# intel/QAT-ZSTD-Plugin

Measured on AMD Instinct MI355X. Metric: input MB/s via ZSTD_compress2 L1 128KiB blocks @1/2/4/8 GPU; ratio vs sw zstd, higher is better.
Workload: dtype u8

## Files before the change

### qat-zstd-plugin_amd/csrc/qzstd_kernels.hip

```cpp
#include <hip/hip_runtime.h>

#include <stdint.h>
#include <stdio.h>
#include <stdlib.h>
#include <string.h>

#include <atomic>
#include <mutex>
#include <sched.h>
#include <time.h>

#include "qzstd_hip.h"
#include "qzstd_hip_internal.h"

#define QZ_PRIO(n) do { if (!CHAIN) __builtin_amdgcn_s_setprio(n); } while (0)

#ifndef QZ_PARSE_SPLIT
#define QZ_PARSE_SPLIT 3
#endif
#ifndef QZ_LINKS_PER_STEP
#define QZ_LINKS_PER_STEP 4
#endif
#ifndef QZ_WAVES_PER_EU
#define QZ_WAVES_PER_EU 5
#endif
#define QZ_OCCUPANCY __attribute__((amdgpu_waves_per_eu(QZ_WAVES_PER_EU)))

#ifdef QZ_DEBUG_DUMP
#define QZ_PLAP(acc) { const u64 tN = __builtin_amdgcn_s_memtime(); acc += tN - tQ; tQ = tN; }
#define QZ_LAP(acc) { const u64 tN = __builtin_amdgcn_s_memtime(); acc += tN - tP; tP = tN; }
#define QZ_CLAP(k) { const u64 tN = __builtin_amdgcn_s_memtime(); dC[k] += tN - tC; tC = tN; }
#else
#define QZ_PLAP(acc)
#define QZ_LAP(acc)
#define QZ_CLAP(k)
#endif

namespace {

constexpr int kMatchWaves = 8;
constexpr int kMatchThreads = kMatchWaves * 64;
constexpr int kThreads = kMatchThreads + 64;
constexpr uint32_t kTileLog = 9;
constexpr uint32_t kTile = 1u << kTileLog;
constexpr uint32_t kWin = kTile >> 6;
constexpr uint32_t kTagBits = 14;
constexpr uint32_t kTagMask = (1u << kTagBits) - 1u;
constexpr uint32_t kPrime1 = 2654435761u;
constexpr uint32_t kPrime2 = 0x85EBCA77u;
constexpr uint32_t kNone = 0xFFFFFFFFu;
constexpr uint32_t kRing = QZ_RING;
constexpr uint32_t kRingMask = kRing - 1u;
constexpr uint32_t kMirror = QZSTD_HIP_RING_MIRROR;
constexpr uint32_t kLook = 4608u;
constexpr uint32_t kNear = kRing - kLook - 3u * kTile - 1024u;
static_assert((kRing & kRingMask) == 0u && kRing >= 16384u, "the ring is a power of two of at least 16 KiB");
constexpr size_t kLdsPerCu = QZSTD_HIP_LDS_MAX;
constexpr uint32_t kEL = QZSTD_HIP_CHAIN_ENTRY_LINKS;
constexpr uint32_t kEQ = QZSTD_HIP_CHAIN_ENTRY_LINKS / 4u;
static_assert(kEL == 4u || kEL == 8u, "chain entries hold four or eight links");
constexpr uint32_t kLdsBase = QZSTD_HIP_LDS_BASE;
constexpr uint32_t kLagT = 2u;

struct LaunchArgs {
    const uint8_t *src;
    const qzstd_hip_block_t *blocks;
    uint4 *seqs;
    uint32_t *nseq;
    qzstd_hip_profile_t prof;
    uint4 *chain;
    uint32_t chainStride;
    uint32_t chainEntries;
    uint32_t pwWords;
    uint32_t orderedLds;
#ifdef QZ_DEBUG_DUMP
    uint32_t dbg;
#endif
};

// ... 613 lines not shown
        stv[k] = (p < nh && p + 4u <= segE) ? (__umulhi(mixH, pf.tableSize) | (((mixH >> 3) & kTagMask) << 16)) : kNone;
    }
    if (ordered) {
#pragma unroll
        for (uint32_t k = 0; k < kWin; k++) {
            const uint32_t mineK = ((t0 + 64u * k + lane + 1u) << kTagBits) | (stv[k] >> 16);
            uint32_t pred = 0u;
            if (stv[k] != kNone) pred = atomicMax(&tbl[stv[k] & 0xFFFFu], mineK);
            P1[64u * k + lane] = pred;
        }
    } else {
#pragma unroll 1
        for (uint32_t k = 0; k < kWin; k++) {
            const uint32_t st = stv[k];
            const bool vk = st != kNone;
            const uint32_t slotK = st & 0xFFFFu;
            const uint32_t mineK = ((t0 + 64u * k + lane + 1u) << kTagBits) | (st >> 16);
            uint32_t prd = 0u, fin = mineK;
            if (vk) {
                uint32_t *e = &tbl[slotK];
                prd = __hip_atomic_load(e, __ATOMIC_RELAXED, __HIP_MEMORY_SCOPE_WORKGROUP);
                atomicMax(e, mineK);
                fin = __hip_atomic_load(e, __ATOMIC_RELAXED, __HIP_MEMORY_SCOPE_WORKGROUP);
            }
            u64 rem = __ballot(fin != mineK);
            uint32_t predLane = lane;
            while (rem) {
                const uint32_t s0 = rdlane(slotK, (uint32_t)__builtin_ctzll(rem));
                const bool in = vk && slotK == s0;
                const u64 grp = __ballot(in);
                const u64 lower = grp & below(lane);
                if (in && lower) predLane = 63u - (uint32_t)__builtin_clzll(lower);
                rem &= ~grp;
            }
            const uint32_t fromLane = (uint32_t)__shfl((int)mineK, (int)predLane);
            P1[64u * k + lane] = vk ? (predLane != lane ? fromLane : prd) : 0u;
        }
    }
}

struct HistShare {
    uint32_t *flags;
    uint32_t item;
    uint32_t epoch;
    uint32_t spinLimit;
    uint32_t nItems;
    uint32_t *tabFlags;
    uint32_t *linkFlags;
    uint32_t *tabs;
};
constexpr uint32_t kSvcTabStride = QZ_CHAIN_TABLE;
static_assert((uint32_t)kMatchWaves * kPvStride <= QZ_CHAIN_TABLE, "the deferred parse's eight windows of parse words must fit in the head table (QZ_CHAIN_TABLE)");

template <bool HAS_LONG, bool REP, bool CHAIN, bool TURNS, bool NEAR, bool DEFER = false>
__device__ __forceinline__ uint32_t qz_item(const LaunchArgs &args, const qzstd_hip_block_t &blk, const uint8_t *gsrc, uint4 *out,
                                            uint4 *chainB, uint32_t *p1B, const HistShare hsh)
{
    extern __shared__ __attribute__((aligned(16))) uint8_t smem[];
    const uint32_t tid = threadIdx.x;
    const uint32_t lane = tid & 63u;
    const uint32_t wave = rdfirst(tid >> 6);
    const bool matcher = wave < (uint32_t)kMatchWaves;
    const uint32_t n = blk.srcLen;
    const qzstd_hip_profile_t pf = args.prof;
    const uint32_t nh = n >= pf.hashBytes ? n - pf.hashBytes + 1u : 0u;
    const uint32_t nTiles = (nh + kTile - 1u) >> kTileLog;
    const uint32_t itEnd = (DEFER && !CHAIN) ? nTiles : nTiles + kLagT;
    static_assert(kNear + kLagT * kTile + 4u <= kRing - kLook, "the ring no longer holds a near source when its tile is parsed / emitted");
    const uint32_t tabShift = (uint32_t)__builtin_clz(pf.tableSize) + 1u, longShift = pf.longSize ? (uint32_t)__builtin_clz(pf.longSize) + 1u : 31u;
    const uint32_t firstTile = blk.parseFrom >> kTileLog;
    if (blk.parseFrom != 0u && (pf.segLog == 0u || (blk.parseFrom & ((1u << pf.segLog) - 1u)) != 0u || blk.parseFrom >= n)) {
        return QZSTD_HIP_NSEQ_ERROR;
    }
    if (NEAR && n > kRing) return QZSTD_HIP_NSEQ_ERROR;
    if (DEFER && args.pwWords != 0u && ((n + kTile - 1u) & ~(kTile - 1u)) > args.pwWords) return QZSTD_HIP_NSEQ_ERROR;
    if (DEFER && CHAIN && args.chainEntries != 0u && ((n + kTile - 1u) & ~(kTile - 1u)) * kEQ > args.chainEntries) return QZSTD_HIP_NSEQ_ERROR;

    uint8_t *smemI = (uint8_t *)(__attribute__((address_space(3))) uint8_t *)kLdsBase;
    if ((uint32_t)(uintptr_t)(__attribute__((address_space(3))) uint8_t *)smem != 0u) {
        return QZSTD_HIP_NSEQ_ERROR;
    }
    uint32_t *ring32 = reinterpret_cast<uint32_t *>(smemI);
    uint4 *ring128 = reinterpret_cast<uint4 *>(smemI);
    uint32_t *tbl = reinterpret_cast<uint32_t *>(smemI + kRing + kMirror);
    uint32_t *tblL = tbl + pf.tableSize;
    uint32_t *nearTab = tblL + pf.longSize;
    uint32_t *srec = nearTab + kTile;
    uint32_t *pv = srec + kLagT * kWin * kSrecWords;
    uint32_t *turnCtr = pv + kLagT * kPvStride;
    uint32_t *P1odd = turnCtr + QZSTD_HIP_LDS_CTRL / 4u;
    const uint4 *g128 = reinterpret_cast<const uint4 *>(gsrc);
    Src src;
    src.ring = (LdsWords)ring32;
    src.g = (HbmWords)reinterpret_cast<const uint32_t *>(gsrc);
    src.nearLimit = NEAR ? 0xFFFFFFFFu : kNear;
    const uint32_t nPad = (n + 15u) & ~15u;

    const uint32_t itBegin = firstTile;
    const uint32_t histEnd = itBegin << kTileLog;
    const uint32_t hi = umin(nPad, histEnd + kLook + (itBegin ? 0u : kTile));
    const uint32_t lo = hi > kRing ? (hi - kRing + 15u) & ~15u : 0u;
    constexpr uint32_t kStep = (uint32_t)kThreads * 16u;
    const uint32_t hashEnd = CHAIN ? 0u : histEnd;
    uint32_t fo = (hashEnd ? 0u : lo) + tid * 16u;
    uint4 fa0 = make_uint4(0u, 0u, 0u, 0u), fb0 = fa0, fa1 = fa0, fb1 = fa0;
    if (fo < hi) { fa0 = g128[fo >> 4]; if (fo < hashEnd) fb0 = g128[(fo >> 4) + 1u]; }
    if (fo + kStep < hi) { fa1 = g128[(fo + kStep) >> 4]; if (fo + kStep < hashEnd) fb1 = g128[((fo + kStep) >> 4) + 1u]; }
    for (uint32_t i = tid; i < pf.tableSize + pf.longSize; i += kThreads) tbl[i] = 0u;
    if (!(CHAIN && itBegin != 0u)) {
        for (uint32_t i = tid; i < kTile; i += kThreads) nearTab[i] = 0xFFFFFFFFu;
// ... 645 lines not shown
                uint32_t P[9], pa[8];
                load_dw_r<9>(src, p + 16u, rp16, false, P);
#pragma unroll
                for (int i = 0; i < 8; i++) pa[i] = __builtin_amdgcn_alignbyte(P[i + 1], P[i], p & 3u);
                if (need1) { const uint32_t l = tail_len(src, pa, q1 + 16u, ring_back(rp16, p - q1), far1); l1 = 16u + l; need1 = l == 32u && 48u < cap; }
                if (HAS_LONG && need3) { const uint32_t l = tail_len(src, pa, q3 + 16u, ring_back(rp16, p - q3), far3); l3 = 16u + l; need3 = l == 32u && 48u < cap; }
                if (need2) { const uint32_t l = tail_len(src, pa, q2 + 16u, ring_back(rp16, p - q2), false); l2 = 16u + l; need2 = l == 32u && 48u < cap; }
            }
            while (need1 || need2 || need3) {
                const int which = need1 ? 1 : (need3 ? 3 : 2);
                const uint32_t q = which == 1 ? q1 : (which == 3 ? q3 : q2);
                const uint32_t L = which == 1 ? l1 : (which == 3 ? l3 : l2);
                const uint32_t l = chunk_len(src, p + L, ring_fwd(rp, L), p - q, which == 1 ? far1 : (which == 3 ? far3 : false));
                const bool more = l == 32u && L + 32u < cap;
                if (which == 1) { l1 = L + l; need1 = more; }
                else if (which == 3) { l3 = L + l; need3 = more; }
                else { l2 = L + l; need2 = more; }
            }
            QZ_PRIO(0);
            l1 = umin(l1, cap); l2 = umin(l2, cap); l3 = umin(l3, cap);
            if (l1 >= 4u) { cl = l1; off = p - q1; }
            if (l3 >= 4u && l3 > cl) { cl = l3; off = p - q3; }
            if (l2 >= 4u && l2 >= cl) { cl = l2; off = p - q2; }
            }
        }
        }
        if (!CHAIN && it < nTiles && !history && !QZ_ABLATED(4u)) write_flags(it, cl, off);
#pragma unroll
        for (uint32_t i = kLagT - 1u; i > 0u; i--) { offH[i] = offH[i - 1u]; lenH[i] = lenH[i - 1u]; }
        offH[0] = off;
        lenH[0] = cl;
        rp = ring_fwd(rp, kTile);
        QZ_LAP(dI2)
        if (DEFER && !CHAIN) QZ_BARRIER_LDS(); else __syncthreads();
        QZ_LAP(dW2)
    }
#ifdef QZ_DEBUG_DUMP
    if (!(blk.mark & QZSTD_HIP_MARK_COMPACT)) {
    if (lane == 0) out[blk.seqCap - 3u - wave] = make_uint4((uint32_t)dI1, (uint32_t)dW1, (uint32_t)dI2, (uint32_t)dW2);
    if (lane == 0) out[blk.seqCap - 24u - 2u * wave] = make_uint4((uint32_t)(dC[0] >> 4), (uint32_t)(dC[1] >> 4), (uint32_t)(dC[2] >> 4), (uint32_t)(dC[3] >> 4));
    if (lane == 0) out[blk.seqCap - 25u - 2u * wave] = make_uint4((uint32_t)(dC[4] >> 4), (uint32_t)dC[5], 0u, 0u);
    if (lane == 0) out[blk.seqCap - 12u - wave] = make_uint4(__builtin_amdgcn_s_getreg((4 << 0) | (0 << 6) | (31 << 11)), 0u, 0u, 0u);
    }
#endif
    if constexpr (!DEFER) return 0u;
    }

    if constexpr (DEFER && !REP) {
        constexpr uint32_t kSegLog = 12u, kSeg = 1u << kSegLog, kMaxSegs = QZSTD_HIP_BLOCK_MAX >> kSegLog;
        static_assert(kMaxSegs <= 64u, "one lane per segment in the prefix step");
        constexpr uint32_t kNoAnchor = 0xFFFFFFFFu;
        uint32_t *segCnt = srec, *segEndA = srec + kMaxSegs;
        const uint32_t firstSeg = blk.parseFrom >> kSegLog, nSegs = (nh + kSeg - 1u) >> kSegLog;
#ifdef QZ_DEBUG_DUMP
        const u64 tD0 = __builtin_amdgcn_s_memtime();
#endif
        if (wave == 0u && lane == 0u) segCnt[2u * kMaxSegs] = firstSeg;
        __syncthreads();
#ifdef QZ_DEBUG_DUMP
        const u64 tD1 = __builtin_amdgcn_s_memtime();
#endif
        {
            const uint32_t S0 = rdfirst(segCnt[2u * kMaxSegs]);
            const uint32_t lastDw = (nPad >> 2) - 1u;
            auto load_tile = [&](uint32_t tb, uint32_t (&dst)[kWin]) {
#pragma unroll
                for (uint32_t j = 0; j < kWin; j++) dst[j] = p1B[tb + 64u * j + lane];
            };
            uint32_t nxt[kWin];
            uint32_t sgN = S0 + wave;
            if (sgN < nSegs) load_tile(sgN << kSegLog, nxt);
            while (sgN < nSegs) {
                const uint32_t sg = sgN;
                sgN = sg + (uint32_t)kMatchWaves;
                const uint32_t segStart = sg << kSegLog;
                u64 *recG = reinterpret_cast<u64 *>(p1B + segStart);
                const uint32_t tEnd = umin(segStart + kSeg, nTiles << kTileLog);
                PlainParse st = { segStart, 0u, kNoAnchor };
                for (uint32_t base = segStart; base < tEnd; base += kTile) {
                    uint32_t wds[kWin];
#pragma unroll
                    for (uint32_t j = 0; j < kWin; j++) wds[j] = nxt[j];
                    const uint32_t nb = base + kTile < tEnd ? base + kTile : sgN << kSegLog;
                    if (base + kTile < tEnd || sgN < nSegs) load_tile(nb, nxt);
                    parse_plain_windows<0, kWin>(pf, src, recG, base, n, lastDw, lane, wds, st);
                }
                if (lane == 0u) { segCnt[sg] = st.cnt; segEndA[sg] = st.endA; }
            }
        }
#ifdef QZ_DEBUG_DUMP
        const u64 tD2 = __builtin_amdgcn_s_memtime();
#endif
        __syncthreads();
#ifdef QZ_DEBUG_DUMP
        const u64 tD3 = __builtin_amdgcn_s_memtime();
#endif
        const bool mine = lane >= firstSeg && lane < nSegs;
        const uint32_t cv = mine ? segCnt[lane] : 0u, ev = mine ? segEndA[lane] : kNoAnchor;
        uint32_t incl = cv, last = ev;
#pragma unroll
        for (uint32_t d = 1; d < kMaxSegs; d <<= 1) {
            const uint32_t ci = (uint32_t)__shfl_up((int)incl, d), li = (uint32_t)__shfl_up((int)last, d);
            if (lane >= d) { incl += ci; if (last == kNoAnchor) last = li; }
        }
        const uint32_t total = rdlane(incl, kMaxSegs - 1u), lastAll = rdlane(last, kMaxSegs - 1u);
        const uint32_t anchorEndAll = lastAll == kNoAnchor ? blk.parseFrom : lastAll;
        {
            for (uint32_t sg = firstSeg + wave; sg < nSegs; sg += (uint32_t)kMatchWaves) {
                const u64 *recG = reinterpret_cast<const u64 *>(p1B + (sg << kSegLog));
                const uint32_t cnt = rdlane(cv, sg), first = rdlane(incl, sg) - cnt;
                uint32_t anchorIn = blk.parseFrom;
                if (sg > 0u) { const uint32_t a = rdlane(last, sg - 1u); if (a != kNoAnchor) anchorIn = a; }
                constexpr uint32_t kU = 4u;
                for (uint32_t k0 = 0; k0 < cnt; k0 += 64u * kU) {
                    u64 r[kU], rp1[kU];
#pragma unroll
                    for (uint32_t u = 0; u < kU; u++) {
                        const uint32_t k = k0 + 64u * u + lane;
                        r[u] = k < cnt ? recG[k] : 0ull;
                        rp1[u] = (k < cnt && k) ? recG[k - 1u] : 0ull;
                    }
                    uint32_t P0[kU], P1[kU], Q0[kU], Q1[kU], lit[kU], maxb[kU];
#pragma unroll
                    for (uint32_t u = 0; u < kU; u++) {
                        const uint32_t k = k0 + 64u * u + lane;
                        const uint32_t pm = (uint32_t)r[u] & 0x1FFFFu, off = (uint32_t)(r[u] >> 17) & 0x1FFFFu;
                        lit[u] = k ? pm - (((uint32_t)rp1[u] & 0x1FFFFu) + ((uint32_t)(rp1[u] >> 34) & 0x1FFFu))
                                   : pm - anchorIn;
                        const uint32_t q = pm - off;
                        maxb[u] = k < cnt ? umin(umin(umin(pf.backExt, lit[u]), q), pm & (kSeg - 1u)) : 0u;
                        P0[u] = P1[u] = Q0[u] = Q1[u] = 0u;
                        if (maxb[u]) {
                            const uint32_t pa = pm >= 4u ? pm - 4u : 0u, qa = q >= 4u ? q - 4u : 0u;
                            P0[u] = src.g[pa >> 2]; P1[u] = src.g[(pa >> 2) + 1u];
                            Q0[u] = src.g[qa >> 2]; Q1[u] = src.g[(qa >> 2) + 1u];
                        }
                    }
#pragma unroll
                    for (uint32_t u = 0; u < kU; u++) {
                        const uint32_t k = k0 + 64u * u + lane;
                        if (k < cnt) {
                            const uint32_t pm = (uint32_t)r[u] & 0x1FFFFu, off = (uint32_t)(r[u] >> 17) & 0x1FFFFu, len = (uint32_t)(r[u] >> 34) & 0x1FFFu;
                            const uint32_t q = pm - off;
                            uint32_t b = 0;
                            if (maxb[u]) {
                                const uint32_t pa = pm >= 4u ? pm - 4u : 0u, qa = q >= 4u ? q - 4u : 0u;
                                uint32_t pb = __builtin_amdgcn_alignbyte(P1[u], P0[u], pa & 3u), qb = __builtin_amdgcn_alignbyte(Q1[u], Q0[u], qa & 3u);
                                if (pm < 4u) pb <<= 8u * (4u - pm);
                                if (q < 4u) qb <<= 8u * (4u - q);
                                const uint32_t x = pb ^ qb;
                                b = umin(x ? (uint32_t)__builtin_clz(x) >> 3 : 4u, maxb[u]);
                            }
                            const uint32_t idx = first + k;
                            if (idx < blk.seqCap) store_entry(out, idx, off, lit[u] - b, len + b, blk.mark);
                        }
                    }
                }
            }
#ifdef QZ_DEBUG_DUMP
            if (lane == 0 && !(blk.mark & QZSTD_HIP_MARK_COMPACT))
                out[blk.seqCap - 44u - wave] = make_uint4((uint32_t)(tD1 - tD0), (uint32_t)(tD2 - tD1), (uint32_t)(tD3 - tD2), (uint32_t)(__builtin_amdgcn_s_memtime() - tD3));
#endif
        }
        if (wave != 0u) return 0u;
        uint32_t count = total + 1u;
        if (lane == 0 && total < blk.seqCap) store_entry(out, total, 0u, n - anchorEndAll, 0u, blk.mark);
        if (count + 1u >= blk.seqCap) count = QZSTD_HIP_NSEQ_ERROR;
        return count;
    }

    if constexpr (DEFER && REP) {
        constexpr uint32_t kSegLog = 12u, kSeg = 1u << kSegLog, kSegsPerQ = kRing >> kSegLog;
        static_assert(kSegsPerQ == (uint32_t)kMatchWaves, "one wave per segment of a quarter");
        constexpr uint32_t kNoAnchor = 0xFFFFFFFFu;
        __syncthreads();
        uint32_t *pvW = tbl + wave * kPvStride;
        uint32_t *ctl = srec;
        const uint32_t firstSeg = blk.parseFrom >> kSegLog, nSegs = (nh + kSeg - 1u) >> kSegLog;
        uint32_t total = 0u, anchorCarry = blk.parseFrom;
        for (uint32_t Q = firstSeg / kSegsPerQ; Q * kSegsPerQ < nSegs; Q++) {
            const uint32_t qs = Q * kRing;
            for (uint32_t o = qs + tid * 16u; o < umin(qs + kRing, nPad); o += (uint32_t)kMatchThreads * 16u) {
                const uint4 v = g128[o >> 4];
                ring128[(o & kRingMask) >> 4] = v;
                if ((o & kRingMask) < kMirror) ring128[(kRing + (o & kRingMask)) >> 4] = v;
            }
            __syncthreads();
            const uint32_t sg = Q * kSegsPerQ + wave;
            const uint32_t segStart = sg << kSegLog;
            u64 *recG = reinterpret_cast<u64 *>(p1B + segStart);
            uint32_t cnt = 0u, endA = kNoAnchor;
            if (sg >= firstSeg && sg < nSegs) {
                const uint32_t tEnd = umin(segStart + kSeg, nTiles << kTileLog);
                uint32_t nxt[kWin];
#pragma unroll
                for (uint32_t j = 0; j < kWin; j++) nxt[j] = p1B[segStart + 64u * j + lane];
                {
                    RepState st = { segStart, segStart, 0u, 0u, 0u, 0u, sg };
                    for (uint32_t base = segStart; base < tEnd; base += kTile) {
#pragma unroll
                        for (uint32_t j = 0; j < kWin; j++) pvW[64u * j + lane] = nxt[j];
                        if (base + kTile < tEnd) {
#pragma unroll
                            for (uint32_t j = 0; j < kWin; j++) nxt[j] = p1B[base + kTile + 64u * j + lane];
                        }
                        parse_rep_span<true>(pf, src, pvW, base, base + kTile, n, nh, lane, st, qs, recG);
                    }
                    cnt = st.nseq;
                    if (cnt) endA = st.anchor;
                }
            }
            if (lane == 0u) { ctl[wave] = cnt; ctl[kSegsPerQ + wave] = endA; }
            __syncthreads();
            {
                const uint32_t cv = lane < 2u * kSegsPerQ ? ctl[lane] : 0u;
                uint32_t before = 0u, all = 0u, anchorIn = anchorCarry, anchorOut = anchorCarry;
#pragma unroll
                for (uint32_t j = 0; j < kSegsPerQ; j++) {
                    const uint32_t c = rdlane(cv, j), a = rdlane(cv, kSegsPerQ + j);
                    if (j < wave) { before += c; if (a != kNoAnchor) anchorIn = a; }
                    all += c;
                    if (a != kNoAnchor) anchorOut = a;
                }
                const uint32_t cnt = rdlane(cv, wave);
                for (uint32_t k0 = 0; k0 < cnt; k0 += 64u) {
                    const uint32_t k = k0 + lane;
                    if (k < cnt) {
                        const u64 r = recG[k];
                        const uint32_t pm = (uint32_t)r & 0x1FFFFu, off = (uint32_t)(r >> 17) & 0x1FFFFu, len = (uint32_t)(r >> 34) & 0x1FFFu;
                        uint32_t lit = pm - anchorIn;
                        if (k) lit = (uint32_t)(r >> 47) & 0x1FFFu;
                        const uint32_t q = pm - off;
                        const uint32_t maxb = umin(umin(umin(pf.backExt, lit), q), pm & (kSeg - 1u));
                        uint32_t b = 0;
                        if (maxb) {
                            const uint32_t pb = rd32u(src, pm - 4u, false);
                            uint32_t qb;
                            if (q < qs + 4u) qb = q >= 4u ? rd32u(src, q - 4u, true) : rd32u(src, 0u, true) << (8u * (4u - q));
                            else qb = rd32u(src, q - 4u, false);
                            const uint32_t x = pb ^ qb;
                            b = umin(x ? (uint32_t)__builtin_clz(x) >> 3 : 4u, maxb);
                        }
                        const uint32_t idx = total + before + k;
                        if (idx < blk.seqCap) store_entry(out, idx, off, lit - b, len + b, blk.mark);
                    }
                }
                total += all;
                anchorCarry = anchorOut;
            }
            __syncthreads();
        }
        if (wave != 0u) return 0u;
        uint32_t count = total + 1u;
        if (lane == 0 && total < blk.seqCap) store_entry(out, total, 0u, n - anchorCarry, 0u, blk.mark);
        if (count + 1u >= blk.seqCap) count = QZSTD_HIP_NSEQ_ERROR;
        return count;
    }
    return 0u;
}

template <bool HAS_LONG, bool REP, bool CHAIN, bool TURNS, bool NEAR>
__global__ __launch_bounds__(kThreads) QZ_OCCUPANCY void qzstd_find_sequences_kernel(LaunchArgs args)
{
    const qzstd_hip_block_t blk = args.blocks[blockIdx.x];
    const uint32_t count = qz_item<HAS_LONG, REP, CHAIN, TURNS, NEAR, true>(args, blk, args.src + blk.srcOff, args.seqs + blk.seqOff,
                                                              CHAIN ? args.chain + (size_t)blockIdx.x * args.chainStride : nullptr,
                                                              reinterpret_cast<uint32_t *>(args.chain + (size_t)blockIdx.x * args.chainStride + args.chainEntries),
                                                              HistShare{ nullptr, 0u, 0u, 0u, 0u, nullptr, nullptr, nullptr });
    asm volatile("s_waitcnt vmcnt(0)" ::: "memory");
    __syncthreads();
    if (threadIdx.x == 0u)
        __hip_atomic_store(args.nseq + blockIdx.x, count, __ATOMIC_RELEASE, __HIP_MEMORY_SCOPE_SYSTEM);
}

constexpr uint32_t kSvcQueue = 4096u;
constexpr uint32_t kSvcRing = 256u;
constexpr uint32_t kSvcMaxItems = 32u;
constexpr uint32_t kSvcSlots = 1024u;
constexpr uint32_t kSvcRejected = 0xFFFFFFFEu;

struct SvcDev {
    u64 items[kSvcQueue][8];
    uint32_t head;
    uint32_t done;
    uint32_t quit;
    uint32_t spinFails;
    uint32_t started;
    uint32_t taken;
    uint32_t pad[2];
    uint32_t sliceFlag[kSvcSlots][kSvcMaxItems];
    uint32_t histFlag[kSvcSlots][kSvcMaxItems];
    uint32_t tabFlag[kSvcSlots][kSvcMaxItems];
    uint32_t linkFlag[kSvcSlots][kSvcMaxItems];
};

struct SvcHost {
    u64 ring[kSvcRing][8];
    uint32_t state;
    uint32_t quitReq;
    u64 consumed;
    u64 itemsDone;
    uint32_t spinFails;
    uint32_t pad;
    u64 dbg[8];
};

typedef __attribute__((address_space(1))) u64 *gu64p;
typedef __attribute__((address_space(1))) uint32_t *gu32p;

__device__ __forceinline__ u64 svc_tag(u64 n, uint32_t entries) { return (n / entries) % 255ull + 1ull; }
__device__ __forceinline__ u64 svc_payload(u64 g) { return g & 0x00FFFFFFFFFFFFFFull; }


constexpr uint32_t kSvcProfiles = 24u;
__device__ __forceinline__ uint32_t svc_profile_index(uint32_t levelByte) { return ((levelByte & 0x7Fu) - 1u) + ((levelByte & 0x80u) ? 12u : 0u); }

template <bool HAS_LONG, bool REP, bool CHAIN, bool TURNS, bool MULTI>
__global__ __launch_bounds__(kThreads) void qzstd_service_worker(LaunchArgs args, SvcDev *sv, uint32_t ctlOff, uint32_t spinLimit, const qzstd_hip_profile_t *profs)
{
    const uint32_t tid = threadIdx.x, lane = tid & 63u;
    const uint32_t wave = rdfirst(tid >> 6);
    uint32_t *ctl = (uint32_t *)(__attribute__((address_space(3))) uint32_t *)(size_t)(kLdsBase + ctlOff);
    if (tid == 0u) (void)__hip_atomic_fetch_add(&sv->started, 1u, QZ_RLX_AGENT);
    for (;;) {
        if (wave == 0u) {
// ... 244 lines not shown
    hipEvent_t bigEv[kBig] = {};
    bool bigUsed[kBig] = {};
    size_t bigLds[kBig] = {};
    int bigNext = 0;
    size_t lds = 0;
    long long launchNs = 0;
    bool sawWorkers = false;
    bool wide = false;
};
Service g_svc[64];
std::atomic<int> g_svcFreeze{0};

struct SvcConfig { int enabled, workers, idleUs, spinLimit; };
const SvcConfig &svc_config()
{
    static const SvcConfig c = [] {
        SvcConfig k;
        const char *e = getenv("QZSTD_HIP_SERVICE"), *w = getenv("QZSTD_HIP_SERVICE_WORKERS"), *i = getenv("QZSTD_HIP_SERVICE_IDLE_US");
        k.enabled = e ? atoi(e) : 1;
        k.workers = w ? atoi(w) : 0;
        k.idleUs = i ? atoi(i) : 20000;
        if (k.idleUs < 100) k.idleUs = 100;
        k.spinLimit = 1 << 20;
        return k;
    }();
    return c;
}

int svc_stop_locked(Service &s, unsigned waitMs)
{
    if (!s.hs) return 0;
    if (__atomic_load_n(&s.hs->state, __ATOMIC_ACQUIRE) != 0u) {
        __atomic_store_n(&s.hs->quitReq, 1u, __ATOMIC_RELEASE);
        struct timespec t0, t;
        clock_gettime(CLOCK_MONOTONIC, &t0);
        while (__atomic_load_n(&s.hs->state, __ATOMIC_ACQUIRE) != 0u) {
            clock_gettime(CLOCK_MONOTONIC, &t);
            if ((t.tv_sec - t0.tv_sec) * 1000ll + (t.tv_nsec - t0.tv_nsec) / 1000000ll > (long long)waitMs) { s.broken = 1; return 1; }
            sched_yield();
        }
    }
    return 0;
}

#define QZ_SEARCHES(X, last)                                                                                    \
    X(false, false, false, false, last), X(false, true, false, false, last),        \
    X(false, false, false, true, last), X(false, true, false, true, last),                \
    X(false, false, true, true, last), X(false, true, true, true, last),      \
    X(true, false, false, false, last), X(true, true, false, false, last)
#define QZ_K(L, R, C, T, N) reinterpret_cast<const void *>(qzstd_find_sequences_kernel<L, R, C, T, N>)
#define QZ_W(L, R, C, T, M) reinterpret_cast<const void *>(qzstd_service_worker<L, R, C, T, M>)
const void *const kLaunchKernels[16] = { QZ_SEARCHES(QZ_K, false), QZ_SEARCHES(QZ_K, true) };
const void *const kWorkers[8] = { QZ_SEARCHES(QZ_W, false) };
#undef QZ_K
#undef QZ_W
#undef QZ_SEARCHES

int variant_index(const qzstd_hip_profile_t &p, bool nearK)
{
    const int search = p.chainDepth ? 2 : (p.longSize ? 3 : (p.subTileLog ? 1 : 0));
    return (nearK ? 8 : 0) + 2 * search + (p.repWin ? 1 : 0);
}

}

SvcFreeze::SvcFreeze()
{
    g_svcFreeze.fetch_add(1);
    for (int d = 0; d < 64; d++) {
        Service &s = g_svc[d];
        if (!s.hs) continue;
        std::lock_guard<std::mutex> g(s.mu);
        (void)svc_stop_locked(s, 2000);
    }
}
SvcFreeze::~SvcFreeze() { g_svcFreeze.fetch_sub(1); }

static int g_ldsOrdered[64];
static std::mutex g_probeMu;

int probe_lds_order(int device, int physDev)
{
    {
        const int known = __atomic_load_n(&g_ldsOrdered[device], __ATOMIC_ACQUIRE);
        if (known > 0) return known - 1;
    }
    std::lock_guard<std::mutex> g(g_probeMu);
    if (g_ldsOrdered[device] > 0) return g_ldsOrdered[device] - 1;
    int verdict = 0;
    const char *force = getenv("QZSTD_HIP_ORDERED_LDS");
    uint32_t *dBad = nullptr, hBad = 1u;
    if (!(force && atoi(force) == 0) && hipSetDevice(physDev) == hipSuccess && hipMalloc(&dBad, sizeof(uint32_t)) == hipSuccess) {
        if (hipMemset(dBad, 0, sizeof(uint32_t)) == hipSuccess) {
            hipLaunchKernelGGL(qzstd_probe_lds_order, dim3(512), dim3(kThreads), 0, 0, dBad);
            if (hipGetLastError() == hipSuccess && hipMemcpy(&hBad, dBad, sizeof(uint32_t), hipMemcpyDeviceToHost) == hipSuccess)
                verdict = hBad == 0u;
        }
        (void)hipFree(dBad);
    }
    (void)hipGetLastError();
    __atomic_store_n(&g_ldsOrdered[device], verdict + 1, __ATOMIC_RELEASE);
    return verdict;
}

extern "C" {

int qzstd_hip_find_sequences(int device, void *stream, int level, const void *d_src,
                             const qzstd_hip_block_t *d_blocks, uint32_t nBlocks, uint32_t maxBlockLen,
                             void *d_seqs, uint32_t *d_nseq, void *d_work, size_t workBytes)
{
    LaunchArgs a;
    if (nBlocks == 0) return 0;
    if (!d_src || !d_blocks || !d_seqs || !d_nseq) return fail_msg("qzstd_hip_find_sequences: null pointer");
    if (maxBlockLen > QZSTD_HIP_BLOCK_MAX) return fail_msg("qzstd_hip_find_sequences: block larger than 128 KiB");
    if (qzstd_hip_profile_for_level(level, maxBlockLen, &a.prof))
        return fail_msg("qzstd_hip_find_sequences: level outside 1..12 (optionally | QZSTD_HIP_LEVEL_REPCODES)");
    if (a.prof.tileLog != kTileLog || a.prof.extLog < 8 || a.prof.extLog > 15 || a.prof.capLen > 48 || a.prof.capLen < 32 ||
        a.prof.minMatch < 4 || a.prof.hashBytes < 4 || a.prof.hashBytes > 8 || a.prof.repWin > 16 || a.prof.chainDepth > 64 ||
        a.prof.lazy > 4 || (a.prof.subTileLog != 0u && a.prof.subTileLog != 6u) || (a.prof.segLog != 0u && (a.prof.segLog < kTileLog || a.prof.segLog > 17u)) ||
        (a.prof.chainDepth && (a.prof.subTileLog != 6u || a.prof.longSize || a.prof.nearTab)) || (a.prof.longSize && a.prof.subTileLog))
        return fail_msg("qzstd_hip_find_sequences: unsupported profile");
    const size_t lds = qzstd_hip_lds_bytes(level, maxBlockLen);
    if (lds == 0) return fail_msg("qzstd_hip_find_sequences: LDS budget exceeded");
    QZ_SET_DEVICE(device);
    bool big = lds + qzstd_hip_lds_bytes(1, QZSTD_HIP_BLOCK_MAX) > kLdsPerCu;
    std::unique_lock<std::mutex> bigLock;
    if (device >= 0 && device < 64) {
        Service &sv = g_svc[device];
        bigLock = std::unique_lock<std::mutex>(sv.mu);
        big = big || sv.wide;
        if (sv.hs && __atomic_load_n(&sv.hs->state, __ATOMIC_ACQUIRE) != 0u && lds + sv.lds > kLdsPerCu) (void)svc_stop_locked(sv, 2000);
    }
    {
        static std::mutex attrMu;
        static bool attrDone[64];
        std::lock_guard<std::mutex> g(attrMu);
        if (phys(device) < 0) return fail_msg("qzstd_hip_find_sequences: device index out of range");
        if (!attrDone[device]) {
            size_t most = 0;
            for (int l = 1; l <= 12; l++) {
                const size_t b = qzstd_hip_lds_bytes(l, QZSTD_HIP_BLOCK_MAX);
                if (b > most) most = b;
            }
            for (const void *f : kLaunchKernels)
                QZ_CHECK(hipFuncSetAttribute(f, hipFuncAttributeMaxDynamicSharedMemorySize, (int)most),
                         "hipFuncSetAttribute(MaxDynamicSharedMemorySize)");
            attrDone[device] = true;
        }
    }
    a.chain = nullptr;
    a.pwWords = 0;
    a.chainStride = 0;
    a.chainEntries = 0;
    a.orderedLds = 0;
    if (a.prof.chainDepth) {
        a.orderedLds = (uint32_t)probe_lds_order(device, phys(device));
        const size_t need = qzstd_hip_workspace_bytes(level, nBlocks, maxBlockLen);
        if (!d_work || workBytes < need) return fail_msg("qzstd_hip_find_sequences: workspace missing or too small (qzstd_hip_workspace_bytes)");
        a.chain = static_cast<uint4 *>(d_work);
        a.chainStride = (uint32_t)(need / nBlocks / sizeof(uint4));
        a.chainEntries = (uint32_t)(need / nBlocks / (4u * QZSTD_HIP_CHAIN_ENTRY_LINKS + 4u)) * kEQ;
    } else {
        const size_t need = qzstd_hip_workspace_bytes(level, nBlocks, maxBlockLen);
        if (!d_work || workBytes < need || need == 0) return fail_msg("qzstd_hip_find_sequences: workspace missing or too small (qzstd_hip_workspace_bytes)");
        a.chain = static_cast<uint4 *>(d_work);
        a.chainStride = (uint32_t)(need / nBlocks / sizeof(uint4));
        a.pwWords = (uint32_t)(need / nBlocks / 33u * 8u);
    }
    if (a.prof.segLog != 12u) return fail_msg("qzstd_hip_find_sequences: unsupported profile (the deferred parse of a launch works on 4 KiB segments)");
    a.src = static_cast<const uint8_t *>(d_src);
    a.blocks = d_blocks;
    a.seqs = static_cast<uint4 *>(d_seqs);
    a.nseq = d_nseq;
#ifdef QZ_DEBUG_DUMP
    { const char *ab = getenv("QZSTD_HIP_ABLATE"); a.dbg = ab ? (uint32_t)atoi(ab) : 0u; }
#endif
#ifdef QZ_DEBUG_DUMP
    size_t ldsLaunch = lds;
    { const char *pad = getenv("QZSTD_HIP_LDS_PAD"); if (pad) ldsLaunch += (size_t)atoi(pad); }
#else
    const size_t ldsLaunch = lds;
#endif
    const dim3 grid(nBlocks), wg(kThreads);
    const void *kernel = kLaunchKernels[variant_index(a.prof, maxBlockLen <= kRing)];
    void *kargs[1] = { &a };
    if (!a.prof.chainDepth && ((a.prof.tableSize & (a.prof.tableSize - 1u)) != 0u || (a.prof.longSize & (a.prof.longSize - 1u)) != 0u || a.prof.hashBytes > 7u))
        return fail_msg("qzstd_hip_find_sequences: unsupported profile (tables below the chain levels are powers of two, hashBytes <= 7)");
    QZ_CHECK(hipLaunchKernel(kernel, grid, wg, kargs, ldsLaunch, (hipStream_t)stream), "launch qzstd_find_sequences_kernel");
    QZ_CHECK(hipGetLastError(), "launch qzstd_find_sequences_kernel");
    if (big && bigLock.owns_lock()) {
        Service &sv = g_svc[device];
        int k = sv.bigNext;
        for (int tries = 0; tries < Service::kBig && sv.bigUsed[k]; tries++) {
            if (hipEventQuery(sv.bigEv[k]) != hipErrorNotReady) { (void)hipGetLastError(); sv.bigUsed[k] = false; break; }
            k = (k + 1) % Service::kBig;
        }
        if (sv.bigUsed[k]) { (void)hipEventSynchronize(sv.bigEv[k]); (void)hipGetLastError(); }
        sv.bigNext = (k + 1) % Service::kBig;
        if (!sv.bigEv[k] && hipEventCreateWithFlags(&sv.bigEv[k], hipEventDisableTiming) != hipSuccess) { sv.bigEv[k] = nullptr; (void)hipGetLastError(); }
        if (sv.bigEv[k] && hipEventRecord(sv.bigEv[k], (hipStream_t)stream) == hipSuccess) { sv.bigUsed[k] = true; sv.bigLds[k] = lds; }
        else (void)hipGetLastError();
    }
    return 0;
}

int qzstd_hip_occupancy(int device, int level)
{
    qzstd_hip_profile_t p;
    if (qzstd_hip_profile_for_level(level, QZSTD_HIP_BLOCK_MAX, &p)) return fail_msg("qzstd_hip_occupancy: bad level");
    const size_t lds = qzstd_hip_lds_bytes(level, QZSTD_HIP_BLOCK_MAX);
    QZ_SET_DEVICE(device);
    const void *k = kLaunchKernels[variant_index(p, false)];
    (void)hipFuncSetAttribute(k, hipFuncAttributeMaxDynamicSharedMemorySize, (int)lds);
    int n = 0;
    QZ_CHECK(hipOccupancyMaxActiveBlocksPerMultiprocessor(&n, k, kThreads, lds), "hipOccupancyMaxActiveBlocksPerMultiprocessor");
    return n;
}

}

namespace {

const void *svc_worker_variant(const qzstd_hip_profile_t &p) { return kWorkers[variant_index(p, false)]; }

int svc_level_index(int level)
{
    const int l = level & ~QZSTD_HIP_LEVEL_REPCODES;
    return (l >= 1 && l <= 12) ? (l - 1) + ((level & QZSTD_HIP_LEVEL_REPCODES) ? 12 : 0) : -1;
}

int svc_launch_locked(int device, Service &s, int level)
{
    const SvcConfig &cfg = svc_config();
    LaunchArgs a;
    memset(&a, 0, sizeof(a));
    if (qzstd_hip_profile_for_level(level, QZSTD_HIP_BLOCK_MAX, &a.prof)) return fail_msg("service: bad level");
    static const bool multiOn = [] { const char *v = getenv("QZSTD_HIP_SERVICE_MULTI"); return !(v && atoi(v) == 0); }();
    const bool multi = multiOn && a.prof.longSize == 0u;
// ... 275 lines not shown
```

### qat-zstd-plugin_amd/host/qatseqprod.c

```c
#ifndef _GNU_SOURCE
#define _GNU_SOURCE
#endif
#include "qatseqprod.h"
#include "qzstd_hip.h"

#include <fcntl.h>
#include <pthread.h>
#include <sched.h>
#include <stdint.h>
#include <stdio.h>
#include <stdlib.h>
#include <string.h>
#include <emmintrin.h>
#include <sys/prctl.h>
#include <sys/syscall.h>
#include <sys/types.h>
#include <time.h>
#include <unistd.h>

#ifndef DEBUGLEVEL
#define DEBUGLEVEL 0
#endif

#define QZ_LEVEL_MIN 1
// ... 1153 lines not shown
        QZ_LOG(1, "device %d: no pinned memory for a batch area: %s\n", dev, qzstd_hip_last_error());
        QZ_HOST_FREE(a->hSrc); QZ_HOST_FREE(a->hDesc); QZ_HOST_FREE(a->hCount); QZ_HOST_FREE(a->hSeqs);
        memset(a, 0, sizeof(*a));
        return -1;
    }
    a->seqsCap = seqs;
    return 0;
}

static int qzAreaOpen(QZSTD_Batcher_T *bt, int level, size_t block)
{
    QZSTD_Area_T *a;
    int k, bare = 0;
    for (k = 0; k < QZ_HB_AREAS && !(bt->area[k].st == QZ_AREA_FREE && bt->area[k].hSrc); k++) bare |= bt->area[k].st == QZ_AREA_FREE;
    if (k >= QZ_HB_AREAS) return bare ? -2 : -1;
    a = &bt->area[k];
    a->lap = (a->lap + 1u) & (gProc.hintCompact ? 0xFFFu : 0xFFFFFFu);
    a->staging = a->parts = 0;
    a->wipe = a->sealed = 0;
    if (a->lap == 0u) {
        a->lap = 1u;
        a->wipe = 1;
        a->staging = 1;
    }
    a->st = QZ_AREA_OPEN;
    a->level = level;
    a->block = block;
    a->nBlocks = a->seen = 0;
    a->srcUsed = a->entUsed = 0;
    a->stream = -1;
    a->stuck = 0;
    bt->open = k;
    return k;
}

static void qzAreaRetire(QZSTD_Batcher_T *bt, int ai)
{
    QZSTD_Area_T *a = &bt->area[ai];
    int k;
    if (a->stuck) qzOrphanArea(a, bt->device, a->stream >= 0 ? bt->str[a->stream].stream : NULL);
    for (k = 0; k < QZ_HB_STREAMS_MAX; k++)
        if (bt->str[k].last == ai && !bt->str[k].stuck) bt->str[k].last = -1;
    a->st = QZ_AREA_FREE;
}

static int qzLaunchArea(QZSTD_Session_T *s, QZSTD_Batcher_T *bt, QZSTD_Area_T *a, QZSTD_BStream_T *q)
{
    const int dev = bt->device;
    const size_t work = qzstd_hip_workspace_bytes(a->level, a->nBlocks, (unsigned int)a->block);
    unsigned long t0;
    int direct, rc;
    if (!q->stream && !(q->stream = qzstd_hip_stream_create(dev))) return -1;
    if (work && !(q->dWork = qzGrowDev(dev, q->dWork, &q->dWorkCap, work))) return -1;
    direct = gProc.hintDirect == 1 || (gProc.hintDirect == 2 && work == 0);
    if (!direct) {
        if (!q->dSrc && !(q->dSrc = (unsigned char *)qzstd_hip_malloc(dev, QZ_HB_SRC_BYTES))) return -1;
        t0 = qzNowNs();
        rc = gProc.hintDirect != 3 ? qzstd_hip_copy_in(dev, q->stream, q->dSrc, a->dvSrc, a->srcUsed)
                                   : qzstd_hip_memcpy_h2d(dev, q->stream, q->dSrc, a->hSrc, a->srcUsed);
        if (s) s->hintCopyCallNs += qzNowNs() - t0;
        if (rc) return -1;
    }
    t0 = qzNowNs();
    rc = qzstd_hip_find_sequences(dev, q->stream, a->level, direct ? a->dvSrc : q->dSrc, (const qzstd_hip_block_t *)a->dvDesc, a->nBlocks,
                                  (unsigned int)a->block, a->dvSeqs, (unsigned int *)a->dvCount, q->dWork, q->dWorkCap);
    if (s) s->hintLaunchCallNs += qzNowNs() - t0;
    if (rc) return -1;
    __atomic_fetch_add(&gProc.devBlocks[dev][0], (unsigned long)a->nBlocks, __ATOMIC_RELAXED);
    __atomic_fetch_add(&bt->launches, 1ul, __ATOMIC_RELAXED);
    __atomic_fetch_add(&bt->blocks, (unsigned long)a->nBlocks, __ATOMIC_RELAXED);
    return 0;
}

static void qzAreaFailCounts(QZSTD_Area_T *a)
{
    memset(a->hCount, 0xFF, a->nBlocks * sizeof(unsigned int));
}

static void qzIssueOpen(QZSTD_Session_T *s, QZSTD_Batcher_T *bt, int force, int want)
{
    const int n = gProc.hintBatches;
    for (;;) {
        const int ai = want >= 0 ? want : bt->open;
        QZSTD_Area_T *a;
        int k, pick = -1, busy = 0, rc, go;
        if (ai < 0) return;
        a = &bt->area[ai];
        if (a->st != QZ_AREA_OPEN || a->nBlocks == 0) return;
        if (a->staging > 0) {
            if (!force) return;
            pthread_cond_wait(&bt->cv, &bt->mu);
            continue;
        }
        go = force || a->sealed;
        for (k = 0; k < n && pick < 0; k++)
            if (qzStreamFree(bt, (bt->nextStream + k) % n)) pick = (bt->nextStream + k) % n;
        for (k = 0; k < n && pick < 0 && go; k++) {
            const int j = (bt->nextStream + k) % n;
            if (bt->str[j].issuing) busy = 1;
            else if (qzStreamUsable(bt, j)) pick = j;
        }
        if (pick < 0 && !go) return;
        if (pick < 0 && busy) {
            pthread_cond_wait(&bt->cv, &bt->mu);
            continue;
        }
        if (bt->open == ai) {
// ... 784 lines not shown
```

Baseline: 22850.

## Split each block's deferred parse across several workgroups with an atomic join

Adds a split kernel that divides one block's plain deferred parse into up to K segment ranges, each run by its own workgroup. Per-segment counts and anchors go to global memory, and the last workgroup to arrive (chosen by an atomic ticket) does the prefix scan and emit. K is picked from occupancy so nBlocks*K does not exceed the number of resident workgroups. This is meant to use idle CUs when there are few blocks, at the cost of an extra memset, global round-trips and fences. The host also changes its direct-source rule so any non-chain level reads the source directly, where before only zero-workspace launches did.

```diff
diff --git a/qat-zstd-plugin_amd/csrc/qzstd_kernels.hip b/qat-zstd-plugin_amd/csrc/qzstd_kernels.hip
--- a/qat-zstd-plugin_amd/csrc/qzstd_kernels.hip
+++ b/qat-zstd-plugin_amd/csrc/qzstd_kernels.hip
@@ -25,6 +25,9 @@
 #define QZ_WAVES_PER_EU 5
 #endif
 #define QZ_OCCUPANCY __attribute__((amdgpu_waves_per_eu(QZ_WAVES_PER_EU)))
+#ifndef QZ_SPLIT_K_MAX
+#define QZ_SPLIT_K_MAX 8u
+#endif
 
 #ifdef QZ_DEBUG_DUMP
 #define QZ_PLAP(acc) { const u64 tN = __builtin_amdgcn_s_memtime(); acc += tN - tQ; tQ = tN; }
@@ -744,10 +747,21 @@
 constexpr uint32_t kSvcTabStride = QZ_CHAIN_TABLE;
 static_assert((uint32_t)kMatchWaves * kPvStride <= QZ_CHAIN_TABLE, "the deferred parse's eight windows of parse words must fit in the head table (QZ_CHAIN_TABLE)");
 
-template <bool HAS_LONG, bool REP, bool CHAIN, bool TURNS, bool NEAR, bool DEFER = false>
+struct SplitJoin {
+    uint32_t *join;
+    uint32_t nItems;
+    uint32_t nFull;
+    uint32_t fromAll;
+};
+constexpr uint32_t kJoinTicket = 0u, kJoinSegs = 16u;
+constexpr uint32_t kJoinWords = kJoinSegs + 2u * (QZSTD_HIP_BLOCK_MAX >> 12);
+constexpr uint32_t kSplitNotLast = 0u;
+
+template <bool HAS_LONG, bool REP, bool CHAIN, bool TURNS, bool NEAR, bool DEFER = false, bool SPLIT = false>
 __device__ __forceinline__ uint32_t qz_item(const LaunchArgs &args, const qzstd_hip_block_t &blk, const uint8_t *gsrc, uint4 *out,
-                                            uint4 *chainB, uint32_t *p1B, const HistShare hsh)
-{
+                                            uint4 *chainB, uint32_t *p1B, const HistShare hsh, const SplitJoin sj = SplitJoin{ nullptr, 1u, 0u, 0u })
+{
+    static_assert(!SPLIT || (DEFER && !REP && !CHAIN), "only the plain deferred parse is split");
     extern __shared__ __attribute__((aligned(16))) uint8_t smem[];
     const uint32_t tid = threadIdx.x;
     const uint32_t lane = tid & 63u;
@@ -1499,6 +1513,9 @@
         constexpr uint32_t kNoAnchor = 0xFFFFFFFFu;
         uint32_t *segCnt = srec, *segEndA = srec + kMaxSegs;
         const uint32_t firstSeg = blk.parseFrom >> kSegLog, nSegs = (nh + kSeg - 1u) >> kSegLog;
+        const uint32_t nAll = SPLIT ? sj.nFull : n, fromAll = SPLIT ? sj.fromAll : blk.parseFrom;
+        const uint32_t firstSegAll = SPLIT ? sj.fromAll >> kSegLog : firstSeg;
+        const uint32_t nSegsAll = SPLIT ? ((sj.nFull >= pf.hashBytes ? sj.nFull - pf.hashBytes + 1u : 0u) + kSeg - 1u) >> kSegLog : nSegs;
 #ifdef QZ_DEBUG_DUMP
         const u64 tD0 = __builtin_amdgcn_s_memtime();
 #endif
@@ -1532,17 +1549,41 @@
                     if (base + kTile < tEnd || sgN < nSegs) load_tile(nb, nxt);
                     parse_plain_windows<0, kWin>(pf, src, recG, base, n, lastDw, lane, wds, st);
                 }
+                if constexpr (SPLIT) {
+                    if (sj.nItems > 1u) {
+                        if (lane == 0u) { sj.join[kJoinSegs + sg] = st.cnt; sj.join[kJoinSegs + kMaxSegs + sg] = st.endA; }
+                    } else if (lane == 0u) { segCnt[sg] = st.cnt; segEndA[sg] = st.endA; }
+                } else
                 if (lane == 0u) { segCnt[sg] = st.cnt; segEndA[sg] = st.endA; }
             }
         }
 #ifdef QZ_DEBUG_DUMP
         const u64 tD2 = __builtin_amdgcn_s_memtime();
 #endif
+        if constexpr (SPLIT) {
+            if (sj.nItems > 1u) {
+                asm volatile("s_waitcnt vmcnt(0)" ::: "memory");
+                __syncthreads();
+                if (tid == 0u) {
+                    __builtin_amdgcn_fence(__ATOMIC_RELEASE, "agent");
+                    asm volatile("s_waitcnt vmcnt(0)" ::: "memory");
+                    const uint32_t ticket = __hip_atomic_fetch_add(sj.join + kJoinTicket, 1u, QZ_RLX_AGENT);
+                    if (ticket + 1u == sj.nItems) {
+                        __builtin_amdgcn_fence(__ATOMIC_ACQUIRE, "agent");
+                        asm volatile("s_waitcnt vmcnt(0)" ::: "memory");
+                    }
+                    segCnt[2u * kMaxSegs] = ticket;
+                }
+                __syncthreads();
+                if (rdfirst(segCnt[2u * kMaxSegs]) + 1u != sj.nItems) return kSplitNotLast;
+                if (tid < 2u * kMaxSegs) segCnt[tid] = sj.join[kJoinSegs + tid];
+            }
+        }
         __syncthreads();
 #ifdef QZ_DEBUG_DUMP
         const u64 tD3 = __builtin_amdgcn_s_memtime();
 #endif
-        const bool mine = lane >= firstSeg && lane < nSegs;
+        const bool mine = lane >= firstSegAll && lane < nSegsAll;
         const uint32_t cv = mine ? segCnt[lane] : 0u, ev = mine ? segEndA[lane] : kNoAnchor;
         uint32_t incl = cv, last = ev;
 #pragma unroll
@@ -1551,12 +1592,12 @@
             if (lane >= d) { incl += ci; if (last == kNoAnchor) last = li; }
         }
         const uint32_t total = rdlane(incl, kMaxSegs - 1u), lastAll = rdlane(last, kMaxSegs - 1u);
-        const uint32_t anchorEndAll = lastAll == kNoAnchor ? blk.parseFrom : lastAll;
+        const uint32_t anchorEndAll = lastAll == kNoAnchor ? fromAll : lastAll;
         {
-            for (uint32_t sg = firstSeg + wave; sg < nSegs; sg += (uint32_t)kMatchWaves) {
+            for (uint32_t sg = firstSegAll + wave; sg < nSegsAll; sg += (uint32_t)kMatchWaves) {
                 const u64 *recG = reinterpret_cast<const u64 *>(p1B + (sg << kSegLog));
                 const uint32_t cnt = rdlane(cv, sg), first = rdlane(incl, sg) - cnt;
-                uint32_t anchorIn = blk.parseFrom;
+                uint32_t anchorIn = fromAll;
                 if (sg > 0u) { const uint32_t a = rdlane(last, sg - 1u); if (a != kNoAnchor) anchorIn = a; }
                 constexpr uint32_t kU = 4u;
                 for (uint32_t k0 = 0; k0 < cnt; k0 += 64u * kU) {
@@ -1611,7 +1652,7 @@
         }
         if (wave != 0u) return 0u;
         uint32_t count = total + 1u;
-        if (lane == 0 && total < blk.seqCap) store_entry(out, total, 0u, n - anchorEndAll, 0u, blk.mark);
+        if (lane == 0 && total < blk.seqCap) store_entry(out, total, 0u, nAll - anchorEndAll, 0u, blk.mark);
         if (count + 1u >= blk.seqCap) count = QZSTD_HIP_NSEQ_ERROR;
         return count;
     }
@@ -1718,6 +1759,39 @@
     __syncthreads();
     if (threadIdx.x == 0u)
         __hip_atomic_store(args.nseq + blockIdx.x, count, __ATOMIC_RELEASE, __HIP_MEMORY_SCOPE_SYSTEM);
+}
+
+template <bool HAS_LONG, bool TURNS, bool NEAR>
+__global__ __launch_bounds__(kThreads) QZ_OCCUPANCY void qzstd_find_sequences_split_kernel(LaunchArgs args, uint32_t K)
+{
+    constexpr uint32_t kSegLog = 12u;
+    const uint32_t b = blockIdx.x / K, item = blockIdx.x - b * K;
+    qzstd_hip_block_t blk = args.blocks[b];
+    const uint32_t nFull = blk.srcLen, fromAll = blk.parseFrom;
+    if ((NEAR && nFull > kRing) || ((nFull + kTile - 1u) & ~(kTile - 1u)) > args.pwWords) {
+        if (item == 0u && threadIdx.x == 0u) __hip_atomic_store(args.nseq + b, QZSTD_HIP_NSEQ_ERROR, __ATOMIC_RELEASE, __HIP_MEMORY_SCOPE_SYSTEM);
+        return;
+    }
+    const uint32_t nhFull = nFull >= args.prof.hashBytes ? nFull - args.prof.hashBytes + 1u : 0u;
+    const uint32_t nSegs = (nhFull + (1u << kSegLog) - 1u) >> kSegLog;
+    uint32_t per = nSegs, nItems = 1u;
+    if (fromAll == 0u && nSegs > 1u) {
+        per = (nSegs + K - 1u) / K;
+        nItems = (nSegs + per - 1u) / per;
+    }
+    if (item >= nItems) return;
+    if (nItems > 1u) {
+        blk.parseFrom = (item * per) << kSegLog;
+        if (item + 1u < nItems) blk.srcLen = ((item + 1u) * per) << kSegLog;
+    }
+    uint32_t *region = reinterpret_cast<uint32_t *>(args.chain + (size_t)b * args.chainStride);
+    const uint32_t count = qz_item<HAS_LONG, false, false, TURNS, NEAR, true, true>(args, blk, args.src + blk.srcOff, args.seqs + blk.seqOff, nullptr, region,
+                                                                                    HistShare{ nullptr, 0u, 0u, 0u, 0u, nullptr, nullptr, nullptr },
+                                                                                    SplitJoin{ region + args.pwWords, nItems, nFull, fromAll });
+    asm volatile("s_waitcnt vmcnt(0)" ::: "memory");
+    __syncthreads();
+    if (threadIdx.x == 0u && count != kSplitNotLast)
+        __hip_atomic_store(args.nseq + b, count, __ATOMIC_RELEASE, __HIP_MEMORY_SCOPE_SYSTEM);
 }
 
 constexpr uint32_t kSvcQueue = 4096u;
@@ -2068,6 +2142,10 @@
 #define QZ_W(L, R, C, T, M) reinterpret_cast<const void *>(qzstd_service_worker<L, R, C, T, M>)
 const void *const kLaunchKernels[16] = { QZ_SEARCHES(QZ_K, false), QZ_SEARCHES(QZ_K, true) };
 const void *const kWorkers[8] = { QZ_SEARCHES(QZ_W, false) };
+#define QZ_S(L, T, N) reinterpret_cast<const void *>(qzstd_find_sequences_split_kernel<L, T, N>)
+const void *const kSplitKernels[2][4] = { { QZ_S(false, false, false), QZ_S(false, true, false), nullptr, QZ_S(true, false, false) },
+                                          { QZ_S(false, false, true), QZ_S(false, true, true), nullptr, QZ_S(true, false, true) } };
+#undef QZ_S
 #undef QZ_K
 #undef QZ_W
 #undef QZ_SEARCHES
@@ -2161,6 +2239,10 @@
             for (const void *f : kLaunchKernels)
                 QZ_CHECK(hipFuncSetAttribute(f, hipFuncAttributeMaxDynamicSharedMemorySize, (int)most),
                          "hipFuncSetAttribute(MaxDynamicSharedMemorySize)");
+            for (const auto &row : kSplitKernels)
+                for (const void *f : row)
+                    if (f) QZ_CHECK(hipFuncSetAttribute(f, hipFuncAttributeMaxDynamicSharedMemorySize, (int)most),
+                                    "hipFuncSetAttribute(MaxDynamicSharedMemorySize)");
             attrDone[device] = true;
         }
     }
@@ -2197,9 +2279,44 @@
 #else
     const size_t ldsLaunch = lds;
 #endif
-    const dim3 grid(nBlocks), wg(kThreads);
+    dim3 grid(nBlocks);
+    const dim3 wg(kThreads);
     const void *kernel = kLaunchKernels[variant_index(a.prof, maxBlockLen <= kRing)];
-    void *kargs[1] = { &a };
+    uint32_t splitK = 1u;
+    void *kargs[2] = { &a, &splitK };
+    if (!a.prof.chainDepth && !a.prof.repWin && maxBlockLen > (1u << 12) && a.pwWords >= 32u * kJoinWords) {
+        const int search = a.prof.longSize ? 3 : (a.prof.subTileLog ? 1 : 0);
+        const void *splitKernel = kSplitKernels[maxBlockLen <= kRing ? 1 : 0][search];
+        const char *e = getenv("QZSTD_HIP_SPLIT_ITEMS");
+        const int forced = e ? atoi(e) : 0;
+        if (forced == 2 || forced == 4 || forced == 8) splitK = (uint32_t)forced;
+        else if (forced == 0) {
+            static std::mutex resMu;
+            static uint32_t resident[64][2][4];
+            uint32_t res = 0u;
+            if (device >= 0 && device < 64) {
+                std::lock_guard<std::mutex> g(resMu);
+                uint32_t &r = resident[device][maxBlockLen <= kRing ? 1 : 0][search];
+                if (!r) {
+                    int perCu = 0, cus = 0;
+                    if (hipOccupancyMaxActiveBlocksPerMultiprocessor(&perCu, splitKernel, kThreads, lds) == hipSuccess &&
+                        hipDeviceGetAttribute(&cus, hipDeviceAttributeMultiprocessorCount, phys(device)) == hipSuccess && perCu > 0 && cus > 0)
+                        r = (uint32_t)perCu * (uint32_t)cus;
+                    else { (void)hipGetLastError(); r = 1u; }
+                }
+                res = r;
+            }
+            const uint32_t segsMax = (maxBlockLen + (1u << 12) - 1u) >> 12;
+            splitK = QZ_SPLIT_K_MAX;
+            while (splitK > 1u && ((uint64_t)nBlocks * splitK > res || splitK / 2u >= segsMax)) splitK /= 2u;
+        }
+        if (splitK > 1u) {
+            QZ_CHECK(hipMemset2DAsync(reinterpret_cast<uint32_t *>(a.chain) + a.pwWords + kJoinTicket, (size_t)a.chainStride * sizeof(uint4), 0, 16u, nBlocks,
+                                      (hipStream_t)stream), "hipMemset2DAsync(split tickets)");
+            kernel = splitKernel;
+            grid = dim3(nBlocks * splitK);
+        }
+    }
     if (!a.prof.chainDepth && ((a.prof.tableSize & (a.prof.tableSize - 1u)) != 0u || (a.prof.longSize & (a.prof.longSize - 1u)) != 0u || a.prof.hashBytes > 7u))
         return fail_msg("qzstd_hip_find_sequences: unsupported profile (tables below the chain levels are powers of two, hashBytes <= 7)");
     QZ_CHECK(hipLaunchKernel(kernel, grid, wg, kargs, ldsLaunch, (hipStream_t)stream), "launch qzstd_find_sequences_kernel");
diff --git a/qat-zstd-plugin_amd/host/qatseqprod.c b/qat-zstd-plugin_amd/host/qatseqprod.c
--- a/qat-zstd-plugin_amd/host/qatseqprod.c
+++ b/qat-zstd-plugin_amd/host/qatseqprod.c
@@ -1229,7 +1229,7 @@
     int direct, rc;
     if (!q->stream && !(q->stream = qzstd_hip_stream_create(dev))) return -1;
     if (work && !(q->dWork = qzGrowDev(dev, q->dWork, &q->dWorkCap, work))) return -1;
-    direct = gProc.hintDirect == 1 || (gProc.hintDirect == 2 && work == 0);
+    direct = gProc.hintDirect == 1 || (gProc.hintDirect == 2 && !qzIsChainLevel(a->level));
     if (!direct) {
         if (!q->dSrc && !(q->dSrc = (unsigned char *)qzstd_hip_malloc(dev, QZ_HB_SRC_BYTES))) return -1;
         t0 = qzNowNs();
```

Measured after the change: 20970. 0.918x the previous value.
